# Darkkey/erlamsa

Hardware: AMD Instinct MI355X
Metric: mutated_MB_per_s (higher is better)
Workload: dtype u8 (byte edits) + f64 (AS183 draws)

## Files before the change

### erlamsa_amd/csrc/eh_fuse_lds.h

```cpp
#pragma once

namespace eh {

constexpr uint32_t FL_NMAX = 8192;
constexpr uint32_t FL_E_WORDS = FL_NMAX / 2;
constexpr uint32_t FL_M_OFF = FL_E_WORDS, FL_M_WORDS = 264;
constexpr uint32_t FL_H_OFF = FL_M_OFF + FL_M_WORDS, FL_H_WORDS = 264;
constexpr uint32_t FL_NONE = 0xFFFFFFFFu;
static_assert(FL_H_OFF + FL_H_WORDS <= EH_FUSE_LDS_WORDS, "g_fuse_lds too small for eh_fuse_lds.h");
constexpr uint32_t FL_CUR = 0x3FFFu, FL_DEAD = 1u << 14, FL_DROPA = 1u << 15, FL_DROPB = 1u << 30, FL_SP = 1u << 31;

struct FlState {
  cbptr A; cbptr B; uint32_t la, lb; bool sym;
  uint32_t n, g, nn;
  uint32_t ghost;
  uint32_t nsp;
  uint32_t multi;
  uint32_t dboff;
  wptr T;
  uint32_t fast, tab_g0, ntomb;
};
struct FlRound { uint32_t w, nn, ghost, nsp, multi; };

EH_DEV uint16_t* fl_E() { return reinterpret_cast<uint16_t*>(g_fuse_lds); }
EH_DEV uint32_t* fl_M() { return g_fuse_lds + FL_M_OFF; }
EH_DEV uint32_t* fl_H() { return g_fuse_lds + FL_H_OFF; }

EH_DEV uint32_t fl_byte(const FlState& st, uint32_t e, bool side, uint32_t s) {
  uint32_t b;
  if (st.dboff != FL_NONE) b = reinterpret_cast<const uint8_t*>(g_fuse_lds)[st.dboff + e + st.g];
  else b = side ? st.B[s + st.g] : st.A[s + st.g];
  return (st.g & 1u) ? 255u - b : b;
}
EH_DEV uint64_t fl_window(uint32_t i, uint32_t* b64) {
  const uint32_t* M = fl_M();
  uint32_t w0 = M[i >> 5], w1 = M[(i >> 5) + 1], w2 = M[(i >> 5) + 2], sh = i & 31u;
  uint64_t lo = ((uint64_t)w1 << 32) | w0;
  uint64_t r = sh ? (lo >> sh) | ((uint64_t)w2 << (64 - sh)) : lo;
  *b64 = sh ? (w2 >> sh) & 1u : w2 & 1u;
  return r;
}
EH_DEV uint32_t fl_next_start(uint32_t j, uint32_t n) {
  const uint32_t* M = fl_M();
  const uint32_t l = (uint32_t)EH_LANE;
  for (uint32_t wbase = j >> 5; wbase * 32u < n; wbase += 64) {
    uint32_t wd = wbase + l;
    uint32_t v = wd * 32u < n ? M[wd] : 0u;
    if (wd == (j >> 5)) v &= ~0u << (j & 31u);
    unsigned long long any = __ballot(v != 0);
    if (any) {
      int src = (int)__builtin_ctzll(any);
      uint32_t vv = (uint32_t)__builtin_amdgcn_readlane((int)v, src);
      uint32_t idx = (wbase + (uint32_t)src) * 32u + (uint32_t)__builtin_ctz(vv);
      return idx < n ? idx : n;
    }
  }
  return n;
}
EH_DEV uint32_t fl_kth_start(uint32_t k, uint32_t n) {
  const uint32_t* M = fl_M();
  const uint32_t l = (uint32_t)EH_LANE;
  uint32_t seen = 0;
  for (uint32_t wbase = 0; wbase * 32u < n; wbase += 64) {
    uint32_t wd = wbase + l;
    uint32_t v = wd * 32u < n ? M[wd] : 0u;
    if (wd * 32u + 32u > n && wd * 32u < n) v &= (1u << (n & 31u)) - 1u;
    uint32_t c = (uint32_t)__popc(v);
    uint32_t inc = wave_incl_scan(c);
    uint32_t tot = (uint32_t)__builtin_amdgcn_readlane((int)inc, 63);
    if (seen + tot > k) {
      unsigned long long hit = __ballot(seen + inc > k);
      int src = (int)__builtin_ctzll(hit);
      uint32_t vv = (uint32_t)__builtin_amdgcn_readlane((int)v, src);
      uint32_t before = seen + (uint32_t)__builtin_amdgcn_readlane((int)(inc - c), src);
      uint32_t r = k - before;
      for (uint32_t t = 0; t < r; t++) vv &= vv - 1u;
      return (wbase + (uint32_t)src) * 32u + (uint32_t)__builtin_ctz(vv);
    }
    seen += tot;
  }
  return n;
}
EH_DEV void fl_clear_bits(uint32_t a, uint32_t b) {
  uint32_t* M = fl_M();
  const uint32_t l = (uint32_t)EH_LANE;
  if (a >= b) return;
  for (uint32_t wbase = a >> 5; wbase <= ((b - 1u) >> 5); wbase += 64) {
    uint32_t wd = wbase + l;
    if (wd <= ((b - 1u) >> 5)) {
      uint32_t lo = wd * 32u, mask = ~0u;
      if (a > lo) mask &= ~0u << (a - lo);
      if (b < lo + 32u) mask &= (1u << (b - lo)) - 1u;
      M[wd] &= ~mask;
    }
  }
  lanes_sync();
}

struct FlVerdict { bool ch, sp, fdrop, tdrop; uint32_t keepA, keepB; };
EH_DEV FlVerdict fl_verdict(bool sym, bool even, uint32_t rf, uint32_t rt, bool hasA, bool hasB) {
  FlVerdict v;
  if (sym) { rt = rf; hasB = hasA; }
  v.fdrop = hasA && (even ? rf == 1u : true);
  v.tdrop = hasB && (even ? rt == 1u : true);
  uint32_t ef = rf - (v.fdrop ? 1u : 0u), et = rt - (v.tdrop ? 1u : 0u);
  v.sp = rf > 0 && ef == 0;
  v.ch = rf > 0 && (v.sp || rt > 0);
  v.keepA = v.ch ? (v.sp ? 1u : ef) : 0u;
  v.keepB = (v.ch && !v.sp && !sym) ? et : 0u;
  return v;
}

EH_DEV void fl_chunk(const FlState& st, uint32_t i, uint32_t m, uint64_t sb, FlRound& o) {
  const uint32_t l = (uint32_t)EH_LANE;
  uint16_t* E = fl_E();
  const bool in = l < m, even = (st.g & 1u) == 0;
  uint32_t e = in ? (uint32_t)E[i + l] : 0u;
  bool side = !st.sym && e >= st.la;
  uint32_t s = side ? e - st.la : e, slen = side ? st.lb : st.la;
  const bool alive = in && s + st.g < slen;
  const bool star = alive && s + st.g == slen - 1u;
  uint32_t bt = alive ? fl_byte(st, e, side, s) : 0u;
  const unsigned long long upto = (2ull << l) - 1ull;
  uint32_t gs = 63u - (uint32_t)__builtin_clzll((sb & upto) | 1ull);
  unsigned long long later = sb & ~upto;
  uint32_t ge = later ? (uint32_t)__builtin_ctzll(later) : m;
  unsigned long long pgm = (ge >= 64 ? ~0ull : ((1ull << ge) - 1ull)) & ~((1ull << gs) - 1ull);
  const unsigned long long am = __ballot(alive);
  unsigned long long eqm = pgm & am, lessm = 0;
#pragma unroll
  for (int bit = 7; bit >= 0; bit--) {
    unsigned long long mb = __ballot(alive && ((bt >> bit) & 1u));
    if ((bt >> bit) & 1u) { lessm |= eqm & ~mb; eqm &= mb; } else eqm &= ~mb;
  }
  if (!alive) { eqm = 0; lessm = 0; }
  unsigned long long amA = __ballot(alive && !side), amB = __ballot(alive && side);
  if (o.w == i && __ballot(in && (!alive || star || eqm != pgm || (!st.sym && ((amA & pgm) == 0 || (amB & pgm) == 0)))) == 0) {
    const unsigned long long nxtb = (sb >> 1) | (1ull << (m - 1u));
    const uint32_t groups = (uint32_t)__popcll(sb);
    o.nn += groups; o.multi += groups - (uint32_t)__popcll(sb & nxtb); o.w += m;
    return;
  }
  unsigned long long smA = __ballot(star && !side), smB = __ballot(star && side);
  FlVerdict v = fl_verdict(st.sym, even, (uint32_t)__popcll(amA & eqm), (uint32_t)__popcll(amB & eqm), (smA & eqm) != 0, (smB & eqm) != 0);
  bool keep = alive && v.ch && (v.sp ? (star && !side) : !((star && !side && v.fdrop) || (star && side && v.tdrop)));
  unsigned long long km = __ballot(keep);
  uint32_t kc = (uint32_t)__popcll(km);
  if (kc == 0) return;
  const unsigned long long below = (1ull << l) - 1ull;
  uint32_t wi = o.w + (uint32_t)__popcll(km & ((1ull << gs) - 1ull)) + (uint32_t)__popcll(km & lessm) + (uint32_t)__popcll(km & eqm & below);
  bool first = keep && (km & eqm & below) == 0;
  unsigned long long fm = __ballot(first);
  unsigned long long gm = __ballot(first && !st.sym && !v.sp && v.keepB == 0);
  unsigned long long spm = __ballot(first && v.sp);
  unsigned long long mm = __ballot(first && (uint32_t)__popcll(km & eqm) > 1u);
  fl_clear_bits(o.w, o.w + kc);
  if (keep) E[wi] = (uint16_t)e;
  if (first) atomicOr(&fl_M()[wi >> 5], 1u << (wi & 31u));
  lanes_sync();
  if (gm) o.ghost = (uint32_t)__builtin_amdgcn_readlane((int)wi, (int)__builtin_ctzll(gm));
  o.nn += (uint32_t)__popcll(fm); o.nsp += (uint32_t)__popcll(spm); o.multi += (uint32_t)__popcll(mm);
  o.w += kc;
}
EH_DEV void fl_singles(const FlState& st, uint32_t i, uint32_t m, FlRound& o) {
  const uint32_t l = (uint32_t)EH_LANE;
  uint16_t* E = fl_E();
  uint32_t e = l < m ? (uint32_t)E[i + l] : 0u;
  bool keep = l < m && e + st.g < st.la;
  unsigned long long km = __ballot(keep);
  uint32_t kc = (uint32_t)__popcll(km);
  if (kc == 0) return;
  if (o.w != i || kc != m) {
    uint32_t wi = o.w + (uint32_t)__popcll(km & ((1ull << l) - 1ull));
    lanes_sync();
    if (keep) E[wi] = (uint16_t)e;
    uint32_t* M = fl_M();
    const uint32_t a = o.w, b = o.w + kc;
    uint32_t wd = (a >> 5) + l;
    if (l < 3 && wd <= ((b - 1u) >> 5)) {
      uint32_t lo = wd * 32u, mask = ~0u;
      if (a > lo) mask &= ~0u << (a - lo);
      if (b < lo + 32u) mask &= (1u << (b - lo)) - 1u;
      M[wd] |= mask;
    }
    lanes_sync();
  }
  o.nn += kc; o.w += kc;
}

#define FL_UNROLL 4
EH_DEV void fl_big(const FlState& st, uint32_t i, uint32_t L, FlRound& o) {
  const uint32_t l = (uint32_t)EH_LANE;
  uint16_t* E = fl_E();
  uint32_t* H = fl_H();
  const bool even = (st.g & 1u) == 0;
  for (uint32_t k = l; k < 260; k += 64) H[k] = 0;
  lanes_sync();
  uint32_t binA = FL_NONE, binB = FL_NONE;
  for (uint32_t base = 0; base < L; base += 64 * FL_UNROLL) {
    uint32_t ev[FL_UNROLL], bv[FL_UNROLL]; bool sv[FL_UNROLL], inv[FL_UNROLL], stv[FL_UNROLL];
#pragma unroll
    for (int u = 0; u < FL_UNROLL; u++) {
      uint32_t idx = base + 64u * (uint32_t)u + l;
      inv[u] = idx < L;
      ev[u] = inv[u] ? (uint32_t)E[i + idx] : 0u;
      sv[u] = !st.sym && ev[u] >= st.la;
    }
#pragma unroll
    for (int u = 0; u < FL_UNROLL; u++) {
      uint32_t s = sv[u] ? ev[u] - st.la : ev[u], slen = sv[u] ? st.lb : st.la;
      bool nonempty = inv[u] && s + st.g < slen;
      stv[u] = nonempty && s + st.g == slen - 1u;
      bv[u] = nonempty ? fl_byte(st, ev[u], sv[u], s) : 256u;
    }
#pragma unroll
    for (int u = 0; u < FL_UNROLL; u++) {
      if (base + 64u * (uint32_t)u >= L) break;
      uint32_t idx = base + 64u * (uint32_t)u + l;
      if (inv[u]) { st.T[idx] = ev[u] | (bv[u] << 16) | (stv[u] ? 1u << 25 : 0u); atomicAdd(&H[bv[u]], sv[u] ? 0x10000u : 1u); }
      unsigned long long sa = __ballot(stv[u] && !sv[u]), sb2 = __ballot(stv[u] && sv[u]);
      if (sa) binA = (uint32_t)__builtin_amdgcn_readlane((int)bv[u], (int)__builtin_ctzll(sa));
      if (sb2) binB = (uint32_t)__builtin_amdgcn_readlane((int)bv[u], (int)__builtin_ctzll(sb2));
    }
  }
  wave_sync();
  uint32_t keepA[4], keepB[4], flg[4], kb = 0, lc = 0, lsp = 0, lmu = 0; bool gh[4];
#pragma unroll
  for (int j = 0; j < 4; j++) {
    uint32_t b = 4u * l + (uint32_t)j, h = H[b];
    FlVerdict v = fl_verdict(st.sym, even, h & 0xFFFFu, h >> 16, b == binA, b == binB);
    keepA[j] = v.keepA; keepB[j] = v.keepB;
    flg[j] = (v.ch ? 0u : FL_DEAD) | (v.fdrop ? FL_DROPA : 0u) | (v.tdrop ? FL_DROPB : 0u) | (v.sp ? FL_SP : 0u);
    gh[j] = v.ch && !st.sym && !v.sp && v.keepB == 0;
    kb += keepA[j] + keepB[j]; lc += v.ch ? 1u : 0u; lsp += v.sp ? 1u : 0u; lmu += (keepA[j] + keepB[j] > 1u) ? 1u : 0u;
  }
  uint32_t inc = wave_incl_scan(kb);
  uint32_t total = (uint32_t)__builtin_amdgcn_readlane((int)inc, 63);
  uint32_t nch = wave_sum(lc);
  if (total == 0) return;
  lanes_sync();
  fl_clear_bits(o.w, o.w + total);
  uint32_t off = o.w + inc - kb;
  uint32_t ghost_here = FL_NONE;
#pragma unroll
  for (int j = 0; j < 4; j++) {
    uint32_t b = 4u * l + (uint32_t)j;
    H[b] = (off & FL_CUR) | (((off + keepA[j]) & FL_CUR) << 16) | flg[j];
    if (keepA[j] + keepB[j] > 0) atomicOr(&fl_M()[off >> 5], 1u << (off & 31u));
    if (gh[j]) ghost_here = off;
    off += keepA[j] + keepB[j];
  }
  unsigned long long ghm = __ballot(ghost_here != FL_NONE);
  if (ghm) o.ghost = (uint32_t)__builtin_amdgcn_readlane((int)ghost_here, (int)__builtin_ctzll(ghm));
  o.nn += nch; o.nsp += wave_sum(lsp); o.multi += wave_sum(lmu);
  lanes_sync();
  for (uint32_t base = 0; base < L; base += 64 * FL_UNROLL) {
    uint32_t tv[FL_UNROLL];
#pragma unroll
    for (int u = 0; u < FL_UNROLL; u++) { uint32_t idx = base + 64u * (uint32_t)u + l; tv[u] = idx < L ? st.T[idx] : (256u << 16); }
#pragma unroll
    for (int u = 0; u < FL_UNROLL; u++) {
      if (base + 64u * (uint32_t)u >= L) break;
      uint32_t e = tv[u] & 0xFFFFu, bt = (tv[u] >> 16) & 511u; bool star = (tv[u] >> 25) & 1u;
      bool side = !st.sym && e >= st.la;
      uint32_t h = bt < 256u ? H[bt] : FL_DEAD;
      bool keep = !(h & FL_DEAD);
      if (keep) {
        if (h & FL_SP) keep = star && !side;
        else keep = !((star && !side && (h & FL_DROPA)) || (star && side && (h & FL_DROPB)));
      }
      uint32_t mk = bt | (side ? 256u : 0u);
      unsigned long long eq = __ballot(keep);
#pragma unroll
      for (int bit = 0; bit < 9; bit++) { unsigned long long mb = __ballot(keep && ((mk >> bit) & 1u)); eq &= ((mk >> bit) & 1u) ? mb : ~mb; }
      uint32_t rank = (uint32_t)__popcll(eq & ((1ull << l) - 1ull)), cnt = (uint32_t)__popcll(eq);
      lanes_sync();
      if (keep) {
        uint32_t cur = side ? (h >> 16) & FL_CUR : h & FL_CUR;
        E[cur + rank] = (uint16_t)e;
        if (rank == 0) atomicAdd(&H[bt], side ? cnt << 16 : cnt);
      }
      lanes_sync();
    }
  }
  o.w += total;
}

EH_DEV uint32_t fl_round(FlState& st) {
  const uint32_t l = (uint32_t)EH_LANE;
  FlRound o; o.w = 0; o.nn = 0; o.ghost = FL_NONE; o.nsp = 0; o.multi = 0;
  if (st.sym && st.multi == 0) {
    uint16_t* E = fl_E();
    uint32_t* H = fl_H();
    if (st.ntomb >= 190u) {
      uint32_t w = 0;
      for (uint32_t base = 0; base < st.n; base += 64) {
        uint32_t e = base + l < st.n ? (uint32_t)E[base + l] : 0xFFFFu;
        unsigned long long km = __ballot(e != 0xFFFFu);
        lanes_sync();
        if (e != 0xFFFFu) E[w + (uint32_t)__popcll(km & ((1ull << l) - 1ull))] = (uint16_t)e;
        w += (uint32_t)__popcll(km);
        lanes_sync();
      }
      st.n = w; st.ntomb = 0; st.fast = 0;
    }
    if (!st.fast || st.g - st.tab_g0 >= 64u) {
      st.fast = 1; st.tab_g0 = st.g;
      if (l < 64) H[l] = FL_NONE;
      lanes_sync();
      for (uint32_t base = 0; base < st.n; base += 64) {
        uint32_t e = base + l < st.n ? (uint32_t)E[base + l] : 0xFFFFu;
        uint32_t d = st.la - st.g - e;
        if (e != 0xFFFFu && d < 64u) H[d] = base + l;
      }
      lanes_sync();
    }
    const uint32_t at = st.g <= st.la ? H[st.g - st.tab_g0] : FL_NONE;
    if (at == FL_NONE) { st.g++; return st.nn; }
    if (st.nn == 1) return 0;
    if (l == 0) { E[at] = 0xFFFFu; H[64u + st.ntomb] = at; }
    lanes_sync();
    st.ntomb++; st.nn--; st.g++;
    return st.nn;
  }
  uint32_t i = 0;
  while (i < st.n) {
    uint32_t b64 = 0;
    uint64_t sb = fl_window(i, &b64);
    uint32_t rest = st.n - i;
    uint32_t m;
    if (rest <= 64) m = rest;
    else {
      uint64_t cand = (sb >> 1) | ((uint64_t)b64 << 63);
      m = cand ? 64u - (uint32_t)__builtin_clzll(cand) : 0u;
    }
    if (rest < 64) sb &= (1ull << rest) - 1ull;
    if (m == 0) {
      uint32_t end = fl_next_start(i + 65, st.n);
      fl_big(st, i, end - i, o);
      i = end;
    } else {
      if (m < 64) sb &= (1ull << m) - 1ull;
      const uint64_t ones = m < 64 ? (1ull << m) - 1ull : ~0ull;
      if (st.sym && sb == ones) fl_singles(st, i, m, o);
      else fl_chunk(st, i, m, sb, o);
      i += m;
    }
  }
  if (o.nn == 0) return 0;
  st.n = o.w; st.nn = o.nn; st.ghost = o.ghost; st.nsp = o.nsp; st.multi = o.multi; st.g++;
  return o.nn;
}

__device__ __noinline__ bool fuse_jump_lds(Ctx&, cbptr A, uint32_t la, cbptr B, uint32_t lb, bool sym, uint32_t* from, uint32_t* tpos, uint32_t* rounds) {
  EH_CTX;
  const uint32_t l = (uint32_t)EH_LANE;
  FlState st;
  st.A = A; st.B = B; st.la = la; st.lb = lb; st.sym = sym;
  const uint32_t n0 = sym ? la : la + lb;
  st.n = n0; st.g = 0; st.nn = 1; st.ghost = FL_NONE; st.nsp = 0; st.multi = n0 > 1 ? 1u : 0u; st.dboff = FL_NONE;
  st.fast = 0; st.tab_g0 = 0; st.ntomb = 0;
  st.T = nullptr;
  if (n0 > 64) { st.T = (wptr)ws_alloc(c, 4ull * n0); if (!st.T) return false; }
  uint16_t* E = fl_E();
  for (uint32_t k = l; k < n0; k += 64) E[k] = (uint16_t)k;
  for (uint32_t k = l; k < FL_M_WORDS; k += 64) fl_M()[k] = k == 0 ? 1u : 0u;
  {
    uint32_t dbytes = sym ? la : la + lb, off = (2u * n0 + 15u) & ~15u;
    if (off + dbytes + 16u <= FL_E_WORDS * 4u) {
      uint8_t* D = reinterpret_cast<uint8_t*>(g_fuse_lds) + off;
      for (uint32_t k = l; k < la; k += 64) D[k] = A[k];
      if (!sym) for (uint32_t k = l; k < lb; k += 64) D[la + k] = B[k];
      st.dboff = off;
    }
  }
  lanes_sync();
  EH_PT0;
  int64_t fuel = 100000;
  uint64_t gen_entries = (uint64_t)la + lb;
  while (true) {
    if (fuel < 0) break;
    if (rng_rand(c.rng, 8) == 0) break;
    if (c.work_budget) {
      c.work += 16ull * gen_entries;
      if (c.work > c.work_budget) { c.status = CASE_BUDGET; return false; }
    }
#ifdef EH_PROF
    const int pslot = (st.sym && st.multi == 0) ? 102 : (st.g == 0 ? 100 : 101);
#endif
    uint32_t nchild = fl_round(st);
    EH_PT(c, pslot);
    if (nchild == 0) break;
    fuel -= (int64_t)nchild;
    gen_entries = sym ? 2ull * (st.n - st.ntomb) : (uint64_t)st.n + st.nsp;
    (*rounds)++;
  }
  const uint32_t par = st.g & 1u;
  uint32_t ni = rng_rand(c.rng, st.nn);
  uint32_t k = par ? st.nn - 1u - ni : ni;
  uint32_t a, b;
  if (st.sym && st.multi == 0) {
    a = k;
    if (st.ntomb) {
      const uint32_t* H = fl_H();
      for (;;) {
        uint32_t cdead = 0;
        for (uint32_t t0 = 0; t0 < st.ntomb; t0 += 64) cdead += (uint32_t)__popcll(__ballot(t0 + l < st.ntomb && H[64u + t0 + l] <= a));
        if (k + cdead == a) break;
        a = k + cdead;
      }
    }
    b = a + 1u;
  } else { a = fl_kth_start(k, st.n); b = fl_next_start(a + 1u, st.n); }
  uint32_t fc = b - a;
  if (!sym) {
    uint32_t cnt = 0;
    for (uint32_t base = a; base < b; base += 64) cnt += (uint32_t)__popcll(__ballot(base + l < b && (uint32_t)E[base + l] < la));
    fc = cnt;
  }
  uint32_t tc = sym ? fc : (b - a) - fc;
  if (c.fp_on) {
    const uint32_t e0 = uni((uint32_t)E[a]), el = uni((uint32_t)E[a + fc - 1u]);
    c.fp_g = st.g; c.fp_keypos = e0;
    c.fp_special = (fc == 1u && e0 + st.g == la) ? 1u : 0u;
    c.fp_bA = (el + st.g == la) ? 1u : 0u;
    c.fp_bB = sym ? c.fp_bA : ((tc > 0 && uni((uint32_t)E[b - 1u]) - la + st.g == lb) ? 1u : 0u);
    EH_PT(c, 103);
    return true;
  }
  bool special_t = false;
  if (!sym && tc == 0 && a != st.ghost) { tc = 1; special_t = true; }
  *from = la; *tpos = lb;
  if (fc > 0) { uint32_t j = rng_rand(c.rng, fc); *from = (uint32_t)E[a + (par ? fc - 1u - j : j)] + st.g; }
  if (tc > 0) {
    uint32_t j = rng_rand(c.rng, tc);
    if (!special_t) { uint32_t idx = sym ? a + (par ? tc - 1u - j : j) : a + fc + (par ? tc - 1u - j : j); uint32_t e = (uint32_t)E[idx]; *tpos = (sym ? e : e - la) + st.g; }
  }
  *from = uni(*from); *tpos = uni(*tpos);
  EH_PT(c, 103);
  return true;
}

}
```

### erlamsa_amd/engine.py

```python
import ctypes as C
import os

import numpy as np

_HERE = os.path.dirname(os.path.abspath(__file__))
LIB_PATH = os.environ.get("ERLAMSA_HIP_LIB") or os.path.join(_HERE, "liberlamsa_hip.so")

EH_ABI_VERSION = 8
EH_FLAG_ORDERED_OUTPUT = 1
EH_FLAG_META_TRACE = 2
EH_FLAG_FUSE_NO_LDS = 4
EH_FLAG_FUSE_NO_REDUCE = 8
EH_FLAG_SGML_NO_REPLAY = 16
EH_FLAG_SGML_NO_LANES = 32
EH_FLAG_NO_COOP = 64

UNIQUE_PIECE_BYTES = 65536

CASE_OK, CASE_CRASHED, CASE_OVERFLOW, CASE_UNSUPPORTED, CASE_ARENA_FULL, CASE_BUDGET = 0, 1, 2, 3, 4, 5

ABI_SYMBOLS = [
    "eh_create", "eh_destroy", "eh_configure", "eh_corpus_upload", "eh_corpus_attach", "eh_fuzz_batch",
    "eh_fuzz_calls", "eh_reserve", "eh_sync", "eh_result_device", "eh_result_download", "eh_result_fetch", "eh_result_totals", "eh_result_summary", "eh_result_occupancy", "eh_result_diag", "eh_result_cycles", "eh_result_peak", "eh_result_meta", "eh_result_write_files", "eh_result_prof", "eh_selftest_movers", "eh_selftest_zlib",
    "eh_last_kernel_ms", "eh_pool_stats", "eh_coop_stats", "eh_kernel_name", "eh_abi_version", "eh_mutator_count", "eh_mutator_name",
    "eh_mutator_default_pri", "eh_mutator_on_gpu", "eh_pattern_count", "eh_pattern_name",
    "eh_pattern_default_pri", "eh_pattern_on_gpu", "eh_strerror", "eh_last_error",
    "eh_coalesce_limits", "eh_submit", "eh_flush", "eh_poll", "eh_cancel",
    "eh_corpus_device", "eh_stream", "eh_host_alloc", "eh_host_free", "eh_selftest_sort_by_priority", "eh_last_error_copy",
    "eh_comm_unique_id", "eh_comm_init", "eh_comm_init_local", "eh_comm_destroy", "eh_corpus_broadcast", "eh_corpus_allgather",
    "eh_corpus_broadcast_local", "eh_device_count", "eh_meta_atom_count", "eh_meta_atom_name", "eh_batch_done",
    "eh_result_digests", "eh_result_unique", "eh_result_download_select", "eh_selftest_unique",
    "eh_profile_add", "eh_profile_count", "eh_fuzz_calls_profiled", "eh_submit_profiled",
]

MAX_PROFILES = 1024


class EhOptions(C.Structure):
    _fields_ = [("abi_version", C.c_uint32), ("mutations", C.c_char_p), ("patterns", C.c_char_p),
                ("generators", C.c_char_p), ("blockscale", C.c_double), ("ssrf_host", C.c_char_p),
                ("ssrf_port", C.c_int32), ("max_case_bytes", C.c_uint64), ("out_capacity", C.c_uint64),
                ("max_case_work", C.c_uint64), ("max_slots", C.c_uint32), ("flags", C.c_uint32), ("big_case_bytes", C.c_uint64),
                ("pool_bytes", C.c_uint64), ("download_chunk_bytes", C.c_uint64), ("fuse_stream_min", C.c_uint64),
                ("sequence_muta", C.c_uint32), ("reserved0", C.c_uint32)]


class EngineError(RuntimeError):
    def __init__(self, code, msg):
        super().__init__("erlamsa_hip error %d: %s" % (code, msg))
        self.code = code


_lib = None


def load_library():
    global _lib
    if _lib is not None:
        return _lib
    import sys
    if "torch" in sys.modules:
        import torch
        if torch.cuda.is_available():
            torch.cuda.init()
    if not os.path.exists(LIB_PATH):
        raise ImportError("%s not built: run `python -c 'import __graft_entry__ as g; g.build()'`" % LIB_PATH)
    lib = C.CDLL(LIB_PATH)
    vp, u64p, i64p, i32p = C.c_void_p, C.POINTER(C.c_uint64), C.POINTER(C.c_int64), C.POINTER(C.c_int32)
    lib.eh_create.argtypes = [C.c_int, C.POINTER(vp)]
    lib.eh_destroy.argtypes = [vp]
    lib.eh_destroy.restype = None
    lib.eh_configure.argtypes = [vp, C.POINTER(EhOptions)]
    lib.eh_corpus_upload.argtypes = [vp, vp, vp, C.c_uint64]
    lib.eh_corpus_attach.argtypes = [vp, vp, vp, C.c_uint64, C.c_uint64]
    lib.eh_fuzz_batch.argtypes = [vp, i64p, C.c_uint64, C.c_uint64, C.c_uint64, vp]
    lib.eh_fuzz_calls.argtypes = [vp, vp, C.c_uint64, C.c_uint64, vp]
    lib.eh_sync.argtypes = [vp]
    lib.eh_batch_done.argtypes = [vp, C.POINTER(C.c_int)]
    lib.eh_reserve.argtypes = [vp, C.c_uint64]
    lib.eh_result_device.argtypes = [vp, C.POINTER(vp), C.POINTER(vp), C.POINTER(vp), C.POINTER(vp), u64p]
    lib.eh_result_download.argtypes = [vp, vp, C.c_uint64, vp, vp]
    lib.eh_result_totals.argtypes = [vp, u64p, u64p, u64p]
    lib.eh_result_fetch.argtypes = [vp, C.c_uint64, vp, C.c_uint64, u64p]
    lib.eh_result_diag.argtypes = [vp, vp, vp]
    lib.eh_result_cycles.argtypes = [vp, vp]
    lib.eh_result_peak.argtypes = [vp, vp]
    lib.eh_result_write_files.argtypes = [vp, C.c_char_p, C.c_uint64, C.c_uint32, u64p, u64p, u64p]
    lib.eh_result_meta.argtypes = [vp, C.c_uint64, vp, C.c_uint64, u64p]
    lib.eh_result_prof.argtypes = [vp, vp]
    lib.eh_selftest_movers.argtypes = [vp, vp, C.c_uint64, vp, C.c_uint32, vp]
    lib.eh_selftest_zlib.argtypes = [vp, C.c_int, vp, C.c_uint64, vp, C.c_uint64, vp, vp]
    lib.eh_result_digests.argtypes = [vp, vp]
    lib.eh_result_unique.argtypes = [vp, vp, u64p, u64p]
    lib.eh_result_download_select.argtypes = [vp, vp, C.c_uint64, vp, C.c_uint64, vp]
    lib.eh_selftest_unique.argtypes = [vp, vp, vp, vp, C.c_uint64, vp, vp]
    lib.eh_last_kernel_ms.argtypes = [vp, C.POINTER(C.c_float)]
    lib.eh_pool_stats.argtypes = [vp, vp]
    lib.eh_result_summary.argtypes = [vp, vp]
    lib.eh_result_occupancy.argtypes = [vp, vp]
    lib.eh_coop_stats.argtypes = [vp, vp]
    lib.eh_coalesce_limits.argtypes = [vp, C.c_uint64, C.c_uint64]
    lib.eh_submit.argtypes = [vp, vp, C.c_uint64, i64p, u64p]
    lib.eh_flush.argtypes = [vp]
    lib.eh_profile_add.argtypes = [vp, C.c_char_p, C.c_char_p, C.c_double, C.POINTER(C.c_uint32)]
    lib.eh_profile_count.argtypes = [vp, C.POINTER(C.c_uint32)]
    lib.eh_fuzz_calls_profiled.argtypes = [vp, vp, vp, C.c_uint64, C.c_uint64, vp]
    lib.eh_submit_profiled.argtypes = [vp, vp, C.c_uint64, i64p, C.c_uint32, u64p]
    lib.eh_meta_atom_name.restype = C.c_char_p
    lib.eh_meta_atom_name.argtypes = [C.c_int]
    lib.eh_comm_unique_id.argtypes = [vp]
    lib.eh_comm_init.argtypes = [vp, vp, C.c_int, C.c_int]
    lib.eh_comm_init_local.argtypes = [vp, C.c_int]
    lib.eh_comm_destroy.argtypes = [vp]
    lib.eh_corpus_broadcast.argtypes = [vp, C.c_int, vp, vp, C.c_uint64]
    lib.eh_corpus_allgather.argtypes = [vp, vp, vp, C.c_uint64]
    lib.eh_corpus_broadcast_local.argtypes = [vp, C.c_int, C.c_int]
    lib.eh_cancel.argtypes = [vp, C.c_uint64]
    lib.eh_poll.argtypes = [vp, C.c_uint64, vp, C.c_uint64, u64p, C.POINTER(C.c_int32)]
    lib.eh_corpus_device.argtypes = [vp, C.POINTER(vp), C.POINTER(vp), u64p, u64p]
    lib.eh_stream.argtypes = [vp, C.POINTER(vp)]
    lib.eh_host_alloc.argtypes = [C.POINTER(vp), C.c_uint64]
    lib.eh_host_free.argtypes = [vp]
    lib.eh_host_free.restype = None
    lib.eh_selftest_sort_by_priority.argtypes = [vp, C.c_uint32, vp]
    lib.eh_kernel_name.restype = C.c_char_p
    lib.eh_abi_version.restype = C.c_uint32
    for f in ("eh_mutator_name", "eh_pattern_name", "eh_strerror"):
        getattr(lib, f).restype = C.c_char_p
        getattr(lib, f).argtypes = [C.c_int]
    lib.eh_last_error.restype = C.c_char_p
    lib.eh_last_error.argtypes = [vp]
    _lib = lib
    return lib


def mutator_table():
    lib = load_library()
    return [(lib.eh_mutator_name(i).decode(), lib.eh_mutator_default_pri(i), bool(lib.eh_mutator_on_gpu(i)))
            for i in range(lib.eh_mutator_count())]


def pattern_table():
    lib = load_library()
    return [(lib.eh_pattern_name(i).decode(), lib.eh_pattern_default_pri(i), bool(lib.eh_pattern_on_gpu(i)))
            for i in range(lib.eh_pattern_count())]


def sort_by_priority(pris):
    p = np.ascontiguousarray(pris, dtype=np.uint32)
    perm = np.zeros(max(len(p), 1), dtype=np.uint32)
    rc = load_library().eh_selftest_sort_by_priority(p.ctypes.data, len(p), perm.ctypes.data)
    if rc != 0:
        raise EngineError(rc, "eh_selftest_sort_by_priority")
    return [int(x) for x in perm[:len(p)]]


def gpu_mutators():
    return [n for n, _, g in mutator_table() if g]


def gpu_patterns():
    return [n for n, _, g in pattern_table() if g]


class Engine:

    def __init__(self, device=0):
        self.lib = load_library()
        h = C.c_void_p()
        rc = self.lib.eh_create(device, C.byref(h))
        if rc != 0:
            raise EngineError(rc, self.lib.eh_strerror(rc).decode())
        self.h = h
        self._keep = []
        self.n_corpus = 0
        self.last_n = 0

    def close(self):
        if self.h:
            self.lib.eh_destroy(self.h)
            self.h = None

    def __del__(self):
        try:
            self.close()
        except Exception:
            pass

    def _chk(self, rc):
        if rc != 0:
            raise EngineError(rc, self.lib.eh_last_error(self.h).decode() or self.lib.eh_strerror(rc).decode())

    def configure(self, mutations=None, patterns=None, generators=None, blockscale=1.0, ssrf_host=None, ssrf_port=0,
                  max_case_bytes=0, out_capacity=0, max_slots=0, flags=0, max_case_work=0, big_case_bytes=0,
                  pool_bytes=0, download_chunk_bytes=0, fuse_stream_min=0, sequence_muta=False):
        o = EhOptions()
        o.sequence_muta = 1 if sequence_muta else 0
        o.abi_version = EH_ABI_VERSION
        o.mutations = mutations.encode() if mutations is not None else None
        o.patterns = patterns.encode() if patterns is not None else None
        o.generators = generators.encode() if generators is not None else None
        o.blockscale = blockscale
        o.ssrf_host = ssrf_host.encode() if ssrf_host else None
        o.ssrf_port = ssrf_port
        o.max_case_bytes = max_case_bytes
        o.big_case_bytes = big_case_bytes
        o.pool_bytes, o.download_chunk_bytes, o.fuse_stream_min = pool_bytes, download_chunk_bytes, fuse_stream_min
        o.out_capacity = out_capacity
        o.max_slots = max_slots
        o.max_case_work = max_case_work
        o.flags = flags
        self._chk(self.lib.eh_configure(self.h, C.byref(o)))

    def upload_corpus(self, data, off):
        data = np.ascontiguousarray(data, dtype=np.uint8)
        off = np.ascontiguousarray(off, dtype=np.uint64)
        n = len(off) - 1
        self._chk(self.lib.eh_corpus_upload(self.h, data.ctypes.data, off.ctypes.data, n))
        self.n_corpus = n

    def attach_corpus(self, d_data_ptr, d_off_ptr, n, nbytes):
        self._chk(self.lib.eh_corpus_attach(self.h, C.c_void_p(d_data_ptr), C.c_void_p(d_off_ptr), n, nbytes))
        self.n_corpus = n

    @staticmethod
    def comm_unique_id():
        lib = load_library()
        buf = (C.c_uint8 * 128)()
        rc = lib.eh_comm_unique_id(buf)
        if rc != 0:
            raise EngineError(rc, lib.eh_strerror(rc).decode() + " (RCCL could not be loaded: EH_RCCL_LIB)")
        return bytes(buf)

    def comm_init(self, unique_id, rank, nranks):
        buf = (C.c_uint8 * 128).from_buffer_copy(unique_id)
        self._chk(self.lib.eh_comm_init(self.h, buf, rank, nranks))

    def comm_destroy(self):
        self._chk(self.lib.eh_comm_destroy(self.h))

    def corpus_broadcast(self, root, data=None, off=None):
        if data is not None:
            data = np.ascontiguousarray(data, dtype=np.uint8)
            off = np.ascontiguousarray(off, dtype=np.uint64)
            self._chk(self.lib.eh_corpus_broadcast(self.h, root, data.ctypes.data, off.ctypes.data, len(off) - 1))
        else:
            self._chk(self.lib.eh_corpus_broadcast(self.h, root, None, None, 0))
        self.n_corpus = self.corpus_device()[2]

    def corpus_allgather(self, data, off):
        data = np.ascontiguousarray(data, dtype=np.uint8)
        off = np.ascontiguousarray(off, dtype=np.uint64)
        self._chk(self.lib.eh_corpus_allgather(self.h, data.ctypes.data, off.ctypes.data, len(off) - 1))
        self.n_corpus = self.corpus_device()[2]

    @staticmethod
    def comm_init_local(engines):
        arr = (C.c_void_p * len(engines))(*[e.h for e in engines])
        rc = engines[0].lib.eh_comm_init_local(arr, len(engines))
        engines[0]._chk(rc)

    @staticmethod
    def corpus_broadcast_local(engines, root=0):
        arr = (C.c_void_p * len(engines))(*[e.h for e in engines])
        rc = engines[0].lib.eh_corpus_broadcast_local(arr, len(engines), root)
        engines[root]._chk(rc)
        for e in engines:
            e.n_corpus = engines[root].n_corpus

    def corpus_device(self):
        d, o, n, nb = C.c_void_p(), C.c_void_p(), C.c_uint64(), C.c_uint64()
        self._chk(self.lib.eh_corpus_device(self.h, C.byref(d), C.byref(o), C.byref(n), C.byref(nb)))
        return d.value, o.value, n.value, nb.value

    def share_corpus(self, other):
        d, o, n, nb = other.corpus_device()
        self.attach_corpus(d, o, n, nb)
        self._keep.append(other)

    def own_stream(self):
        s = C.c_void_p()
        self._chk(self.lib.eh_stream(self.h, C.byref(s)))
        return s.value or 0

    def fuzz_batch(self, seed=(1, 2, 3), first_case=1, corpus_first=0, n=None, stream=0):
        if n is None:
            n = self.n_corpus - corpus_first
        s = (C.c_int64 * 3)(*seed)
        self._chk(self.lib.eh_fuzz_batch(self.h, s, first_case, corpus_first, n, C.c_void_p(stream)))
        self.last_n = n

    def fuzz_calls(self, seeds, profiles=None, corpus_first=0, stream=0):
        seeds = np.ascontiguousarray(seeds, dtype=np.int64).reshape(-1)
        n = seeds.size // 3
        if profiles is None:
            self._chk(self.lib.eh_fuzz_calls(self.h, seeds.ctypes.data, corpus_first, n, C.c_void_p(stream)))
        else:
            ids = np.ascontiguousarray(profiles, dtype=np.uint32).reshape(-1)
            if ids.size != n:
                raise ValueError("fuzz_calls: %d profile ids for %d seeds" % (ids.size, n))
            self._chk(self.lib.eh_fuzz_calls_profiled(self.h, seeds.ctypes.data, ids.ctypes.data, corpus_first, n, C.c_void_p(stream)))
        self.last_n = n

    def profile_add(self, mutations=None, patterns=None, blockscale=1.0):
        pid = C.c_uint32()
        self._chk(self.lib.eh_profile_add(self.h, mutations.encode() if mutations is not None else None,
                                          patterns.encode() if patterns is not None else None, float(blockscale), C.byref(pid)))
        return pid.value

    def profile_count(self):
        n = C.c_uint32()
        self._chk(self.lib.eh_profile_count(self.h, C.byref(n)))
        return n.value

    def reserve(self, max_cases):
        self._chk(self.lib.eh_reserve(self.h, max_cases))

    def sync(self):
# ... 248 lines not shown
```

### include/erlamsa_hip.h

```cpp
#ifndef ERLAMSA_HIP_H
#define ERLAMSA_HIP_H
#include <stdint.h>
#ifdef __cplusplus
extern "C" {
#endif

#define EH_ABI_VERSION 8

typedef struct eh_ctx eh_ctx;

enum eh_error {
  EH_OK = 0,
  EH_E_INVALID = -1,
  EH_E_NODEVICE = -2,
  EH_E_HIP = -3,
  EH_E_NOMEM = -4,
  EH_E_STATE = -5,
  EH_E_UNSUPPORTED = -6,
  EH_E_AGAIN = -7
};

enum eh_case_status {
  EH_CASE_OK = 0,
  EH_CASE_CRASHED = 1,
  EH_CASE_OVERFLOW = 2,
  EH_CASE_UNSUPPORTED = 3,
  EH_CASE_ARENA_FULL = 4,
  EH_CASE_BUDGET = 5
};

typedef struct eh_options {
  uint32_t abi_version;
  const char* mutations;
  const char* patterns;
  const char* generators;
  double blockscale;
  const char* ssrf_host;
  int32_t ssrf_port;
  uint64_t max_case_bytes;
  uint64_t out_capacity;
  uint64_t max_case_work;
  uint32_t max_slots;
  uint32_t flags;
  uint64_t big_case_bytes;
  uint64_t pool_bytes;
  uint64_t download_chunk_bytes;
  uint64_t fuse_stream_min;
  uint32_t sequence_muta;
  uint32_t reserved0;
} eh_options;

#define EH_FLAG_NO_COOP 64u
#define EH_FLAG_TREE_NO_LANES 128u
#define EH_FLAG_ORDERED_OUTPUT 1u
#define EH_FLAG_META_TRACE 2u
#define EH_FLAG_SGML_NO_LANES 32u
#define EH_FLAG_SGML_NO_REPLAY 16u
#define EH_FLAG_FUSE_NO_REDUCE 8u
#define EH_FLAG_FUSE_NO_LDS 4u

int eh_create(int device, eh_ctx** out);
void eh_destroy(eh_ctx* ctx);
int eh_configure(eh_ctx* ctx, const eh_options* opts);

int eh_corpus_upload(eh_ctx* ctx, const uint8_t* data, const uint64_t* off, uint64_t n);
int eh_corpus_attach(eh_ctx* ctx, const void* d_data, const void* d_off, uint64_t n, uint64_t nbytes);

int eh_device_count(void);
int eh_comm_unique_id(uint8_t id[128]);
int eh_comm_init(eh_ctx* ctx, const uint8_t id[128], int rank, int nranks);
int eh_comm_init_local(eh_ctx** ctxs, int nctx);
int eh_comm_destroy(eh_ctx* ctx);
int eh_corpus_broadcast(eh_ctx* ctx, int root, const uint8_t* data, const uint64_t* off, uint64_t n);
int eh_corpus_allgather(eh_ctx* ctx, const uint8_t* data, const uint64_t* off, uint64_t n_local);
int eh_corpus_broadcast_local(eh_ctx** ctxs, int nctx, int root);

int eh_corpus_device(eh_ctx* ctx, const void** d_data, const void** d_off, uint64_t* n, uint64_t* nbytes);

int eh_stream(eh_ctx* ctx, void** stream);

int eh_host_alloc(void** p, uint64_t bytes);
void eh_host_free(void* p);

int eh_reserve(eh_ctx* ctx, uint64_t max_cases);

int eh_fuzz_batch(eh_ctx* ctx, const int64_t seed[3], uint64_t first_case, uint64_t corpus_first, uint64_t n,
                  void* stream);
int eh_fuzz_calls(eh_ctx* ctx, const int64_t* seeds, uint64_t corpus_first, uint64_t n, void* stream);
int eh_sync(eh_ctx* ctx);
int eh_batch_done(eh_ctx* ctx, int* done);

int eh_coalesce_limits(eh_ctx* ctx, uint64_t flush_cases, uint64_t flush_bytes);
int eh_submit(eh_ctx* ctx, const uint8_t* data, uint64_t len, const int64_t seed[3], uint64_t* ticket);
int eh_flush(eh_ctx* ctx);
int eh_poll(eh_ctx* ctx, uint64_t ticket, uint8_t* out, uint64_t cap, uint64_t* out_len, int32_t* status);
int eh_cancel(eh_ctx* ctx, uint64_t ticket);

#define EH_MAX_PROFILES 1024
int eh_profile_add(eh_ctx* ctx, const char* mutations, const char* patterns, double blockscale, uint32_t* id);
int eh_profile_count(eh_ctx* ctx, uint32_t* n);
int eh_fuzz_calls_profiled(eh_ctx* ctx, const int64_t* seeds, const uint32_t* profile, uint64_t corpus_first, uint64_t n, void* stream);
int eh_submit_profiled(eh_ctx* ctx, const uint8_t* data, uint64_t len, const int64_t seed[3], uint32_t profile, uint64_t* ticket);

int eh_result_device(eh_ctx* ctx, const uint8_t** d_data, const uint64_t** d_off, const uint64_t** d_len,
                     const int32_t** d_status, uint64_t* total_bytes);
int eh_result_download(eh_ctx* ctx, uint8_t* data, uint64_t cap, uint64_t* off, int32_t* status);
int eh_result_fetch(eh_ctx* ctx, uint64_t i, uint8_t* buf, uint64_t cap, uint64_t* out_len);
int eh_result_totals(eh_ctx* ctx, uint64_t* in_bytes, uint64_t* out_bytes, uint64_t* n_cases);
int eh_result_summary(eh_ctx* ctx, uint64_t* out);
int eh_result_occupancy(eh_ctx* ctx, uint64_t* out);
int eh_result_diag(eh_ctx* ctx, uint64_t* draws, int32_t* last_mutator);

int eh_result_cycles(eh_ctx* ctx, uint64_t* cycles);

int eh_result_write_files(eh_ctx* ctx, const char* name_template, uint64_t first_number, uint32_t threads,
                          uint64_t* files_written, uint64_t* bytes_written, uint64_t* not_written);

int eh_meta_atom_count(void);
const char* eh_meta_atom_name(int id);
int eh_result_meta(eh_ctx* ctx, uint64_t i, uint8_t* buf, uint64_t cap, uint64_t* n_events);

#define EH_UNIQUE_PIECE_BYTES 65536
int eh_result_digests(eh_ctx* ctx, uint64_t* digest);
int eh_result_unique(eh_ctx* ctx, uint64_t* first_of, uint64_t* n_unique, uint64_t* unique_bytes);
int eh_result_download_select(eh_ctx* ctx, const uint64_t* idx, uint64_t m, uint8_t* data, uint64_t cap, uint64_t* off);
int eh_selftest_unique(eh_ctx* ctx, const uint8_t* data, const uint64_t* off, const int32_t* status, uint64_t n,
                       uint64_t* digest, uint64_t* first_of);

int eh_result_peak(eh_ctx* ctx, uint64_t* peak);

int eh_result_prof(eh_ctx* ctx, uint64_t* prof);

int eh_selftest_movers(eh_ctx* ctx, uint8_t* buf, uint64_t buf_len, const uint32_t* jobs, uint32_t njobs, uint32_t* eq_out);
int eh_selftest_zlib(eh_ctx* ctx, int op, const uint8_t* in, uint64_t n, uint8_t* out, uint64_t cap, uint64_t* out_len, int32_t* ok);

int eh_selftest_sort_by_priority(const uint32_t* pri, uint32_t n, uint32_t* perm);

int eh_pool_stats(eh_ctx* ctx, uint64_t* out);
int eh_coop_stats(eh_ctx* ctx, uint64_t* out);

int eh_last_kernel_ms(eh_ctx* ctx, float* ms);
const char* eh_kernel_name(void);

uint32_t eh_abi_version(void);
int eh_mutator_count(void);
const char* eh_mutator_name(int id);
int eh_mutator_default_pri(int id);
int eh_mutator_on_gpu(int id);
int eh_pattern_count(void);
const char* eh_pattern_name(int id);
int eh_pattern_default_pri(int id);
int eh_pattern_on_gpu(int id);
const char* eh_strerror(int code);
const char* eh_last_error(eh_ctx* ctx);
uint64_t eh_last_error_copy(eh_ctx* ctx, char* buf, uint64_t cap);

#ifdef __cplusplus
}
#endif
#endif
```

Before: 79730.

## Add pair-group fast path, byte prefetch and lighter bit clears in LDS fuse rounds

Adds a specialized fl_pairs path for windows whose groups all have at most two members, comparing partners with a single shuffle instead of an 8-step ballot radix compare. Prefetches the next chunk's element indices and source bytes from global memory before processing the current chunk, so the load latency overlaps work. Also switches to a bounded three-lane bit-clear and splits the 32-bit halves in the general compare loop. The older behaviour stays available behind a new PLAIN flag. Profiling counters per step kind are added under EH_PROF/HIPEMU.

```diff
diff --git a/erlamsa_amd/csrc/eh_fuse_lds.h b/erlamsa_amd/csrc/eh_fuse_lds.h
--- a/erlamsa_amd/csrc/eh_fuse_lds.h
+++ b/erlamsa_amd/csrc/eh_fuse_lds.h
@@ -19,8 +19,25 @@
   uint32_t dboff;
   wptr T;
   uint32_t fast, tab_g0, ntomb;
+  bool plain;
 };
-struct FlRound { uint32_t w, nn, ghost, nsp, multi; };
+enum { FL_K_SINGLES = 0, FL_K_PAIRS = 1, FL_K_GENERAL = 2, FL_K_BIG = 3 };
+#if defined(EH_PROF) || defined(HIPEMU)
+#define FL_COUNTING 1
+#define FL_STEP(o, k) ((o).steps[k]++)
+#else
+#define FL_STEP(o, k) do { } while (0)
+#endif
+#ifdef HIPEMU
+extern "C" { inline unsigned long long eh_emu_fuse_steps[8] = {0, 0, 0, 0, 0, 0, 0, 0}; }
+#endif
+struct FlRound {
+  uint32_t w, nn, ghost, nsp, multi;
+#ifdef FL_COUNTING
+  uint32_t steps[4];
+#endif
+};
+struct FlPre { bool have; uint32_t e, b; };
 
 EH_DEV uint16_t* fl_E() { return reinterpret_cast<uint16_t*>(g_fuse_lds); }
 EH_DEV uint32_t* fl_M() { return g_fuse_lds + FL_M_OFF; }
@@ -31,6 +48,20 @@
   if (st.dboff != FL_NONE) b = reinterpret_cast<const uint8_t*>(g_fuse_lds)[st.dboff + e + st.g];
   else b = side ? st.B[s + st.g] : st.A[s + st.g];
   return (st.g & 1u) ? 255u - b : b;
+}
+EH_DEV uint32_t fl_byte_of(const FlState& st, const FlPre& pre, uint32_t e, bool side, uint32_t s) {
+  if (!pre.have) return fl_byte(st, e, side, s);
+  return (st.g & 1u) ? 255u - pre.b : pre.b;
+}
+EH_DEV void fl_prefetch(const FlState& st, uint32_t j, FlPre& pre) {
+  const uint32_t l = (uint32_t)EH_LANE;
+  const bool in = j + l < st.n;
+  uint32_t e = in ? (uint32_t)fl_E()[j + l] : 0u;
+  bool side = !st.sym && e >= st.la;
+  uint32_t s = side ? e - st.la : e, slen = side ? st.lb : st.la;
+  uint32_t b = 0;
+  if (in && s + st.g < slen) b = side ? st.B[s + st.g] : st.A[s + st.g];
+  pre.have = true; pre.e = e; pre.b = b;
 }
 EH_DEV uint64_t fl_window(uint32_t i, uint32_t* b64) {
   const uint32_t* M = fl_M();
@@ -96,6 +127,18 @@
   }
   lanes_sync();
 }
+EH_DEV void fl_clear_span(uint32_t a, uint32_t b) {
+  uint32_t* M = fl_M();
+  const uint32_t l = (uint32_t)EH_LANE;
+  uint32_t wd = (a >> 5) + l;
+  if (l < 3 && wd <= ((b - 1u) >> 5)) {
+    uint32_t lo = wd * 32u, mask = ~0u;
+    if (a > lo) mask &= ~0u << (a - lo);
+    if (b < lo + 32u) mask &= (1u << (b - lo)) - 1u;
+    M[wd] &= ~mask;
+  }
+  lanes_sync();
+}
 
 struct FlVerdict { bool ch, sp, fdrop, tdrop; uint32_t keepA, keepB; };
 EH_DEV FlVerdict fl_verdict(bool sym, bool even, uint32_t rf, uint32_t rt, bool hasA, bool hasB) {
@@ -111,16 +154,17 @@
   return v;
 }
 
-EH_DEV void fl_chunk(const FlState& st, uint32_t i, uint32_t m, uint64_t sb, FlRound& o) {
+EH_DEV void fl_chunk(const FlState& st, uint32_t i, uint32_t m, uint64_t sb, const FlPre& pre, FlRound& o) {
   const uint32_t l = (uint32_t)EH_LANE;
   uint16_t* E = fl_E();
   const bool in = l < m, even = (st.g & 1u) == 0;
-  uint32_t e = in ? (uint32_t)E[i + l] : 0u;
+  FL_STEP(o, FL_K_GENERAL);
+  uint32_t e = in ? (pre.have ? pre.e : (uint32_t)E[i + l]) : 0u;
   bool side = !st.sym && e >= st.la;
   uint32_t s = side ? e - st.la : e, slen = side ? st.lb : st.la;
   const bool alive = in && s + st.g < slen;
   const bool star = alive && s + st.g == slen - 1u;
-  uint32_t bt = alive ? fl_byte(st, e, side, s) : 0u;
+  uint32_t bt = alive ? fl_byte_of(st, pre, e, side, s) : 0u;
   const unsigned long long upto = (2ull << l) - 1ull;
   uint32_t gs = 63u - (uint32_t)__builtin_clzll((sb & upto) | 1ull);
   unsigned long long later = sb & ~upto;
@@ -128,10 +172,24 @@
   unsigned long long pgm = (ge >= 64 ? ~0ull : ((1ull << ge) - 1ull)) & ~((1ull << gs) - 1ull);
   const unsigned long long am = __ballot(alive);
   unsigned long long eqm = pgm & am, lessm = 0;
-#pragma unroll
-  for (int bit = 7; bit >= 0; bit--) {
-    unsigned long long mb = __ballot(alive && ((bt >> bit) & 1u));
-    if ((bt >> bit) & 1u) { lessm |= eqm & ~mb; eqm &= mb; } else eqm &= ~mb;
+  if (st.plain) {
+#pragma unroll
+    for (int bit = 7; bit >= 0; bit--) {
+      unsigned long long mb = __ballot(alive && ((bt >> bit) & 1u));
+      if ((bt >> bit) & 1u) { lessm |= eqm & ~mb; eqm &= mb; } else eqm &= ~mb;
+    }
+  } else {
+    uint32_t eql = (uint32_t)eqm, eqh = (uint32_t)(eqm >> 32), lsl = 0, lsh = 0;
+    const bool wide = m > 32u;
+#pragma unroll
+    for (int bit = 7; bit >= 0; bit--) {
+      const unsigned long long mb = __ballot(alive && ((bt >> bit) & 1u));
+      const uint32_t B = 0u - ((bt >> bit) & 1u);
+      const uint32_t nl = eql & ~((uint32_t)mb ^ B);
+      lsl |= (eql ^ nl) & B; eql = nl;
+      if (wide) { const uint32_t nh = eqh & ~((uint32_t)(mb >> 32) ^ B); lsh |= (eqh ^ nh) & B; eqh = nh; }
+    }
+    eqm = ((unsigned long long)eqh << 32) | eql; lessm = ((unsigned long long)lsh << 32) | lsl;
   }
   if (!alive) { eqm = 0; lessm = 0; }
   unsigned long long amA = __ballot(alive && !side), amB = __ballot(alive && side);
@@ -154,7 +212,7 @@
   unsigned long long gm = __ballot(first && !st.sym && !v.sp && v.keepB == 0);
   unsigned long long spm = __ballot(first && v.sp);
   unsigned long long mm = __ballot(first && (uint32_t)__popcll(km & eqm) > 1u);
-  fl_clear_bits(o.w, o.w + kc);
+  if (st.plain) fl_clear_bits(o.w, o.w + kc); else fl_clear_span(o.w, o.w + kc);
   if (keep) E[wi] = (uint16_t)e;
   if (first) atomicOr(&fl_M()[wi >> 5], 1u << (wi & 31u));
   lanes_sync();
@@ -162,9 +220,57 @@
   o.nn += (uint32_t)__popcll(fm); o.nsp += (uint32_t)__popcll(spm); o.multi += (uint32_t)__popcll(mm);
   o.w += kc;
 }
+EH_DEV void fl_pairs(const FlState& st, uint32_t i, uint32_t m, uint64_t sb, const FlPre& pre, FlRound& o) {
+  const uint32_t l = (uint32_t)EH_LANE;
+  uint16_t* E = fl_E();
+  const bool in = l < m, even = (st.g & 1u) == 0;
+  FL_STEP(o, FL_K_PAIRS);
+  uint32_t e = in ? (pre.have ? pre.e : (uint32_t)E[i + l]) : 0u;
+  bool side = !st.sym && e >= st.la;
+  uint32_t s = side ? e - st.la : e, slen = side ? st.lb : st.la;
+  const bool alive = in && s + st.g < slen;
+  const bool star = alive && s + st.g == slen - 1u;
+  uint32_t bt = alive ? fl_byte_of(st, pre, e, side, s) : 0u;
+  const unsigned long long nxtb = (sb >> 1) | (1ull << (m - 1u));
+  const bool isstart = (sb >> l) & 1ull, last = (nxtb >> l) & 1ull;
+  const bool paired = in && !(isstart && last);
+  const uint32_t p = paired ? (isstart ? l + 1u : l - 1u) : l;
+  const uint32_t px = (uint32_t)__shfl((int)((alive ? 1u : 0u) | (side ? 2u : 0u) | (star ? 4u : 0u) | (bt << 3)), (int)p);
+  const bool pal = paired && (px & 1u), pside = (px & 2u) != 0, pstar = pal && (px & 4u);
+  const uint32_t pbt = px >> 3;
+  const bool same = alive && pal && pbt == bt;
+  const uint32_t rf = (alive && !side ? 1u : 0u) + (same && !pside ? 1u : 0u), rt = (alive && side ? 1u : 0u) + (same && pside ? 1u : 0u);
+  if (o.w == i && __ballot(in && (!alive || star || (paired && !same) || (!st.sym && (rf == 0 || rt == 0)))) == 0) {
+    const uint32_t groups = (uint32_t)__popcll(sb);
+    o.nn += groups; o.multi += groups - (uint32_t)__popcll(sb & nxtb); o.w += m;
+    return;
+  }
+  FlVerdict v = fl_verdict(st.sym, even, rf, rt, (star && !side) || (same && pstar && !pside), (star && side) || (same && pstar && pside));
+  bool keep = alive && v.ch && (v.sp ? (star && !side) : !((star && !side && v.fdrop) || (star && side && v.tdrop)));
+  unsigned long long km = __ballot(keep);
+  uint32_t kc = (uint32_t)__popcll(km);
+  if (kc == 0) return;
+  const bool pk = paired && ((km >> p) & 1ull);
+  const bool both = keep && pk && pbt == bt;
+  const uint32_t gs = isstart ? l : l - 1u;
+  uint32_t wi = o.w + (uint32_t)__popcll(km & ((1ull << gs) - 1ull)) + ((pk && (pbt < bt || (pbt == bt && p < l))) ? 1u : 0u);
+  bool first = keep && !(both && p < l);
+  unsigned long long fm = __ballot(first);
+  unsigned long long gm = __ballot(first && !st.sym && !v.sp && v.keepB == 0);
+  unsigned long long spm = __ballot(first && v.sp);
+  unsigned long long mm = __ballot(first && both);
+  fl_clear_span(o.w, o.w + kc);
+  if (keep) E[wi] = (uint16_t)e;
+  if (first) atomicOr(&fl_M()[wi >> 5], 1u << (wi & 31u));
+  lanes_sync();
+  if (gm) o.ghost = (uint32_t)__builtin_amdgcn_readlane((int)wi, (int)__builtin_ctzll(gm));
+  o.nn += (uint32_t)__popcll(fm); o.nsp += (uint32_t)__popcll(spm); o.multi += (uint32_t)__popcll(mm);
+  o.w += kc;
+}
 EH_DEV void fl_singles(const FlState& st, uint32_t i, uint32_t m, FlRound& o) {
   const uint32_t l = (uint32_t)EH_LANE;
   uint16_t* E = fl_E();
+  FL_STEP(o, FL_K_SINGLES);
   uint32_t e = l < m ? (uint32_t)E[i + l] : 0u;
   bool keep = l < m && e + st.g < st.la;
   unsigned long long km = __ballot(keep);
@@ -194,6 +300,7 @@
   uint16_t* E = fl_E();
   uint32_t* H = fl_H();
   const bool even = (st.g & 1u) == 0;
+  FL_STEP(o, FL_K_BIG);
   for (uint32_t k = l; k < 260; k += 64) H[k] = 0;
   lanes_sync();
   uint32_t binA = FL_NONE, binB = FL_NONE;
@@ -286,9 +393,12 @@
   o.w += total;
 }
 
-EH_DEV uint32_t fl_round(FlState& st) {
+EH_DEV uint32_t fl_round(Ctx& c, FlState& st) {
   const uint32_t l = (uint32_t)EH_LANE;
   FlRound o; o.w = 0; o.nn = 0; o.ghost = FL_NONE; o.nsp = 0; o.multi = 0;
+#ifdef FL_COUNTING
+  for (int k = 0; k < 4; k++) o.steps[k] = 0;
+#endif
   if (st.sym && st.multi == 0) {
     uint16_t* E = fl_E();
     uint32_t* H = fl_H();
@@ -324,6 +434,9 @@
     return st.nn;
   }
   uint32_t i = 0;
+  const bool ahead = !st.plain && st.dboff == FL_NONE;
+  FlPre pre; pre.have = false; pre.e = 0; pre.b = 0;
+  if (ahead) fl_prefetch(st, 0, pre);
   while (i < st.n) {
     uint32_t b64 = 0;
     uint64_t sb = fl_window(i, &b64);
@@ -339,14 +452,29 @@
       uint32_t end = fl_next_start(i + 65, st.n);
       fl_big(st, i, end - i, o);
       i = end;
+      if (ahead && i < st.n) fl_prefetch(st, i, pre);
     } else {
       if (m < 64) sb &= (1ull << m) - 1ull;
       const uint64_t ones = m < 64 ? (1ull << m) - 1ull : ~0ull;
+      FlPre nxt; nxt.have = false; nxt.e = 0; nxt.b = 0;
+      if (ahead && i + m < st.n) fl_prefetch(st, i + m, nxt);
+      const uint64_t clr = ~sb & ones;
       if (st.sym && sb == ones) fl_singles(st, i, m, o);
-      else fl_chunk(st, i, m, sb, o);
+      else if (!st.plain && (clr & (clr >> 1)) == 0) fl_pairs(st, i, m, sb, pre, o);
+      else fl_chunk(st, i, m, sb, pre, o);
+      pre = nxt;
       i += m;
     }
   }
+#ifdef FL_COUNTING
+  if (l == 0) for (int k = 0; k < 4; k++) if (o.steps[k]) {
+#ifdef HIPEMU
+    eh_emu_fuse_steps[(st.g >= 2u ? 4 : 0) + k] += o.steps[k];
+#else
+    atomicAdd(&c.p->prof[2 * (44 + k)], (unsigned long long)o.steps[k]); atomicAdd(&c.p->prof[2 * (44 + k) + 1], 1ull);
+#endif
+  }
+#endif
   if (o.nn == 0) return 0;
   st.n = o.w; st.nn = o.nn; st.ghost = o.ghost; st.nsp = o.nsp; st.multi = o.multi; st.g++;
   return o.nn;
@@ -360,6 +488,7 @@
   const uint32_t n0 = sym ? la : la + lb;
   st.n = n0; st.g = 0; st.nn = 1; st.ghost = FL_NONE; st.nsp = 0; st.multi = n0 > 1 ? 1u : 0u; st.dboff = FL_NONE;
   st.fast = 0; st.tab_g0 = 0; st.ntomb = 0;
+  st.plain = (c.p->flags & EH_FLAG_FUSE_LDS_PLAIN) != 0;
   st.T = nullptr;
   if (n0 > 64) { st.T = (wptr)ws_alloc(c, 4ull * n0); if (!st.T) return false; }
   uint16_t* E = fl_E();
@@ -388,7 +517,7 @@
 #ifdef EH_PROF
     const int pslot = (st.sym && st.multi == 0) ? 102 : (st.g == 0 ? 100 : 101);
 #endif
-    uint32_t nchild = fl_round(st);
+    uint32_t nchild = fl_round(c, st);
     EH_PT(c, pslot);
     if (nchild == 0) break;
     fuel -= (int64_t)nchild;
diff --git a/erlamsa_amd/engine.py b/erlamsa_amd/engine.py
--- a/erlamsa_amd/engine.py
+++ b/erlamsa_amd/engine.py
@@ -14,6 +14,8 @@
 EH_FLAG_SGML_NO_REPLAY = 16
 EH_FLAG_SGML_NO_LANES = 32
 EH_FLAG_NO_COOP = 64
+EH_FLAG_TREE_NO_LANES = 128
+EH_FLAG_FUSE_LDS_PLAIN = 256
 
 UNIQUE_PIECE_BYTES = 65536
 
diff --git a/include/erlamsa_hip.h b/include/erlamsa_hip.h
--- a/include/erlamsa_hip.h
+++ b/include/erlamsa_hip.h
@@ -52,6 +52,7 @@
 
 #define EH_FLAG_NO_COOP 64u
 #define EH_FLAG_TREE_NO_LANES 128u
+#define EH_FLAG_FUSE_LDS_PLAIN 256u
 #define EH_FLAG_ORDERED_OUTPUT 1u
 #define EH_FLAG_META_TRACE 2u
 #define EH_FLAG_SGML_NO_LANES 32u
```

After: 78940. -1.0%, worse.
